# rajan-dubey8/camouflage-multimodal

Measured on AMD Instinct MI355X. Metric: images/sec fwd+bwd (fusion model train step: fwd + loss + bwd + clip + AdamW), higher is better.
Workload: dtype bf16; 1 GPU; BASELINE configs[1] on the path that exists (SURVEY 8d): cross-attention fusion model, packed variable-Nr minibatch (Nr ~ real 303..530 histogram, mean 483), Nk=13 real KG rows, train mode dropout 0.3, random-init weights; batch_per_gpu=16, global_batch=16, rg_dim=128, hidden_dim=256, num_heads=8, parallelism=dp1, precision=bf16 MFMA operands, fp32 accumulate/optimizer

## Files before the change

### camouflage_multimodal_amd/csrc/fused_rows.h

```cpp
#pragma once
#include "common.h"

typedef unsigned short us16;

struct ShadowJob { us16* dst; int N, K, transposed, nsrc; const float* src[4]; int rows[4]; int ld[4]; int chunk_begin; int lo; };
#define SHADOW_MAXJ 24
#define SHADOW_MAXZ 24
struct ShadowBatch { ShadowJob j[SHADOW_MAXJ]; int n; void* zero_ptr[SHADOW_MAXZ]; size_t zero_bytes[SHADOW_MAXZ]; int nzero; };
int launch_weight_shadows(ShadowBatch& sb, hipStream_t stream);

struct FrontStream {
  const float* X; int M;
  const us16* W0; const float* b0;
  const us16* W1; const float* bq; const float* bkv;
  us16* X16;
  us16* R16; us16* Q16; us16* KV16;
  int tile_begin;
};
#define FUSED_FRONT_MAXZ 4
#define FUSED_FRONT_MAXX 20
#define FUSED_BWD1_MAXZ 16
struct FrontArgs {
  FrontStream s[2]; float qscale; int save; unsigned long long* stamps; int exp;
  void* zero_ptr[FUSED_FRONT_MAXZ]; unsigned zero_bytes[FUSED_FRONT_MAXZ]; int nzero;
// ... 55 lines not shown

struct Bwd2Args {
  const us16* Q2_16; const us16* dO2_16; const float* lse2; const float* delta2;
  const us16* KV2_16;
  us16* dQKV16;
  const us16* dU16; const us16* WcRgT; us16* dR16;
  float* dQ2acc;
  const float* dKV;
  const us16* dU2_16; const us16* WcKgT; us16* dQKVkg16; us16* dG16;
  float* dGpart;
  int* tickets;
  const int* off; const int* tile_off; const int4* tile_desc;
  int B, Nk, rg_tiles_max, rows_rg; float qscale; DropCfg drop; unsigned long long* stamps;
  int param_space;
  int split_finish;
};
int launch_fused_bwd2(Bwd2Args& a, int variant, hipStream_t stream);
int launch_wide2_bwd2(Bwd2Args& a, hipStream_t stream);
size_t fused_bwd2_lds();

#define FUSED_PART_FLOATS 544
#define FUSED_MAX_SPLITS 64
size_t fused_front_lds();
size_t fused_back_lds();

#define FUSED_WIDE_MAXSEG 48
int launch_wide_front(FrontArgs& a, int rt, hipStream_t stream, int kg_only = 0);
int launch_wide_rgfwd(const FrontStream& f, float qscale, BackArgs& b, int rt, int max_nr, hipStream_t stream);
int launch_wide_back(BackArgs& a, int rt, int max_nr, hipStream_t stream);
int wide_max_rows(int rt);

// ... 4 lines not shown
```

### camouflage_multimodal_amd/csrc/fused_rows.hip

```cpp
#include "fused_rows.h"
#include "shadow_inl.h"
#include "gemm.h"
#include "mfma_inl.h"

namespace {

template <int NT, int KS, bool W_IS_A, int DEPTH, bool USE_ROT = true>
struct Stage {
  static constexpr int TOTAL = NT * KS;
  static constexpr int D = DEPTH < TOTAL ? DEPTH : TOTAL;
  static_assert(!USE_ROT || (KS & (KS - 1)) == 0, "rotated k order: power-of-two k steps");
  u32x4 buf[D];
  const u32x4* wp; int rot;
  __device__ __forceinline__ int keff(int ks) const { return USE_ROT ? ((ks + rot) & (KS - 1)) : ks; }
  __device__ __forceinline__ const u32x4* wptr(int i) const { return wp + 64 * (keff(i / NT) * NT + (i % NT)); }
  __device__ __forceinline__ void prefetch(const u32x4* __restrict__ wp_, int rot_) {
    wp = wp_; rot = rot_;
#pragma unroll
    for (int i = 0; i < D; ++i) buf[i] = *wptr(i);
  }
  __device__ __forceinline__ void run(const char* act, f32x16 (&acc)[NT]) {
    run_f([&](int ks) { return *reinterpret_cast<const bf16x8*>(act + 32 * ks); }, acc);
  }
  template <class F>
// ... 343 lines not shown
      const float il = invL[hd * 16 + j];
      *reinterpret_cast<u32x2*>(bufO + j * PR + 2 * (32 * hd + 4 * f4)) =
          u32x2{pack2(acc[it][0] * il, acc[it][1] * il), pack2(acc[it][2] * il, acc[it][3] * il)};
    }
  }
}

template <int DEPTH, bool ROT, int OCC>
__global__ __launch_bounds__(256, OCC) void back_kernel(const BackArgs a) {
  extern __shared__ __attribute__((aligned(16))) char smem[];
  const int tid = threadIdx.x, lane = tid & 63, l31 = lane & 31, h = lane >> 5;
  const int w = __builtin_amdgcn_readfirstlane(tid >> 6);
  const int nkg = a.B * a.max_splits;
  const int vid = (int)blockIdx.x < a.lead_tiles ? nkg + (int)blockIdx.x : ((int)blockIdx.x < a.lead_tiles + nkg ? (int)blockIdx.x - a.lead_tiles : (int)blockIdx.x);
  const bool kg = vid < nkg;
  const int rot = ROT ? (int)(blockIdx.x >> 3) : 0;
  using L = BackL<OCC>;
  char* bufO = smem + L::O; char* bufY = smem + L::Y;
  float* red = reinterpret_cast<float*>(smem + L::RED);
  float* tile32 = reinterpret_cast<float*>(smem);
  int b; size_t rowg0; int nrows; float inv_n;
  stamp(a.stamps, 0);
  const BackStream& S = a.s[kg ? 1 : 0];
  Stage<2, 16, true, DEPTH> sto;
  Stage<4, 16, false, DEPTH> stf;
  if (!kg) sto.prefetch(reinterpret_cast<const u32x4*>(S.Wo) + (size_t)w * (16 * 2 * 64) + lane, rot);
  if (kg) {
    b = vid / a.max_splits;
    const int sp = vid - b * a.max_splits;
    const int nsplit = (a.off[b + 1] - a.off[b] + SPLIT_ROWS - 1) / SPLIT_ROWS;
    if (sp >= nsplit) return;
    attn_kg_split(a, smem, b, sp, w, lane);
    stamp(a.stamps, 4);
    asm volatile("s_waitcnt vmcnt(0)" ::: "memory");
    __syncthreads();
    int* flag = reinterpret_cast<int*>(red);
    if (tid == 0) flag[0] = __hip_atomic_fetch_add(a.tickets + b, 1, __ATOMIC_RELAXED, __HIP_MEMORY_SCOPE_AGENT);
    __syncthreads();
    stamp(a.stamps, 5);
    if (flag[0] != nsplit - 1) return;
    if (tid == 0) {
      __builtin_amdgcn_fence(__ATOMIC_ACQUIRE, "agent");
      asm volatile("s_waitcnt vmcnt(0)" ::: "memory");
    }
// ... 491 lines not shown
    se.prefetch(reinterpret_cast<const u32x4*>(a.WcKgT) + (size_t)w * (48 * 2 * 64) + 64 * (16 * 2) + lane, 0);
    for (int c = tid; c < 32 * 64; c += 256) {
      const int j = c >> 6, ch = c & 63;
      u32x4 v = u32x4{0u, 0u, 0u, 0u};
      if (j < Nk) {
        const float* src = a.dKV + (krow0 + j) * 512 + 8 * ch;
        const float4 x0 = *reinterpret_cast<const float4*>(src), x1 = *reinterpret_cast<const float4*>(src + 4);
        v = u32x4{pack2(x0.x, x0.y), pack2(x0.z, x0.w), pack2(x1.x, x1.y), pack2(x1.z, x1.w)};
      }
      *reinterpret_cast<u32x4*>(bufT + j * PQ + 512 + 16 * ch) = v;
    }
    __syncthreads();
    f32x16 acc[2] = {zero16(), zero16()};
    se.run(bufT + l31 * PQ + 512 + 16 * h, acc);
    copy_out<6>(bufT, PQ, 512, a.dQKVkg16 + 256, 768, krow0, Nk);
    if (l31 < Nk) {
#pragma unroll
      for (int t = 0; t < 2; ++t)
#pragma unroll
        for (int g = 0; g < 4; ++g) {
          const int c0 = 64 * w + 32 * t + 8 * g + 4 * h;
          const u32x2 uv = *reinterpret_cast<const u32x2*>(a.dU2_16 + (krow0 + l31) * 256 + c0);
          float* dst = a.dGpart + (krow0 + l31) * 256 + c0;
          __hip_atomic_store(dst, acc[t][4 * g] + bf_lo(uv.x), __ATOMIC_RELAXED, __HIP_MEMORY_SCOPE_AGENT);
          __hip_atomic_store(dst + 1, acc[t][4 * g + 1] + bf_hi(uv.x), __ATOMIC_RELAXED, __HIP_MEMORY_SCOPE_AGENT);
          __hip_atomic_store(dst + 2, acc[t][4 * g + 2] + bf_lo(uv.y), __ATOMIC_RELAXED, __HIP_MEMORY_SCOPE_AGENT);
          __hip_atomic_store(dst + 3, acc[t][4 * g + 3] + bf_hi(uv.y), __ATOMIC_RELAXED, __HIP_MEMORY_SCOPE_AGENT);
        }
    }
  } else {
  const int4 td = a.tile_desc[(int)blockIdx.x - a.B];
// ... 103 lines not shown
    sr.run(bufT + l31 * PQ + 16 * h, acc);
    copy_out<6>(bufT, PQ, 512, a.dQKV16 + 256, 768, rowg0, nrows);
    if (rok) {
#pragma unroll
      for (int t = 0; t < 2; ++t)
#pragma unroll
        for (int g = 0; g < 4; ++g) {
          const int c0 = 64 * w + 32 * t + 8 * g + 4 * h;
          const u32x2 uv = *reinterpret_cast<const u32x2*>(a.dU16 + (rowg0 + l31) * 256 + c0);
          *reinterpret_cast<u32x2*>(a.dR16 + (rowg0 + l31) * 256 + c0) =
              u32x2{pack2(acc[t][4 * g] + bf_lo(uv.x), acc[t][4 * g + 1] + bf_hi(uv.x)), pack2(acc[t][4 * g + 2] + bf_lo(uv.y), acc[t][4 * g + 3] + bf_hi(uv.y))};
        }
    }
  }
  stamp(a.stamps, 2);
  }
  asm volatile("s_waitcnt vmcnt(0)" ::: "memory");
  __syncthreads();
  if (tid == 0) flag[0] = __hip_atomic_fetch_add(a.tickets + b, 1, __ATOMIC_RELAXED, __HIP_MEMORY_SCOPE_AGENT);
  __syncthreads();
  if (flag[0] != a.tile_off[b + 1] - a.tile_off[b]) return;
  Stage<2, 16, true, DEPTH, false> sg;
  sg.prefetch(reinterpret_cast<const u32x4*>(a.WcKgT) + (size_t)w * (48 * 2 * 64) + lane, 0);
  if (tid == 0) {
    __builtin_amdgcn_fence(__ATOMIC_ACQUIRE, "agent");
    asm volatile("s_waitcnt vmcnt(0)" ::: "memory");
  }
  __syncthreads();
  const size_t krow0 = (size_t)b * Nk;
  for (int c = tid; c < 32 * 32; c += 256) {
// ... 305 lines not shown
  const int prof = gemm_prof_open(stream, 2.0 * rows * (512.0 * 256.0 + 256.0 * 256.0) + (kg_only ? 0.0 : 10.0 * (double)a.rows_rg * a.Nk * 256.0), PROF_BWD1);
  if (variant == 0) launch_lds<bwd1_kernel<12, false>>(grid, dim3(256), W_LDS, stream, k);
  else              launch_lds<bwd1_kernel<12, true>>(grid, dim3(256), W_LDS, stream, k);
  gemm_prof_close(prof, stream);
  return (int)hipGetLastError();
}

size_t fused_bwd2_lds() { return X_LDS; }

int launch_fused_bwd2(Bwd2Args& a, int variant, hipStream_t stream) {
  (void)variant;
  if (a.B < 1 || a.Nk < 1 || a.Nk > 16 || a.rg_tiles_max < 1 || !a.Q2_16 || !a.dO2_16 || !a.lse2 || !a.delta2 || !a.KV2_16 || !a.dQKV16 ||
      !a.dU16 || !a.WcRgT || !a.dR16 || !a.dQ2acc || !a.dKV || !a.dU2_16 || !a.WcKgT || !a.dQKVkg16 || !a.dG16 || !a.dGpart || !a.tickets || !a.off || !a.tile_off || !a.tile_desc)
    return (int)hipErrorInvalidValue;
  if (!al16(a.dQKV16) || !al16(a.dQKVkg16) || !al16(a.WcRgT) || !al16(a.WcKgT) || !al16(a.dQ2acc) || !al16(a.dKV)) return (int)hipErrorInvalidValue;
  const double rows = (double)a.rows_rg + (double)a.B * a.Nk;
  const int prof = gemm_prof_open(stream, (a.param_space ? 0.0 : 2.0 * rows * 768.0 * 256.0) + 10.0 * (double)a.rows_rg * a.Nk * 256.0, PROF_BWD2);
  if (!a.param_space) a.split_finish = 0;
  if (!a.param_space) launch_lds<bwd2_kernel<12, false>>(dim3(a.B + a.rg_tiles_max), dim3(256), X_LDS, stream, a);
  else                launch_lds<bwd2p_kernel<12, false>>(dim3(a.B + a.rg_tiles_max), dim3(256), X_LDS, stream, a);
  if (a.split_finish) hipLaunchKernelGGL(bwd2_finish_kernel, dim3(a.B), dim3(256), 0, stream, a);
  gemm_prof_close(prof, stream);
  return (int)hipGetLastError();
}
```

### camouflage_multimodal_amd/csrc/fusion_abi.hip

```cpp
#include <hip/hip_runtime.h>

#include <algorithm>
#include <cmath>
#include <cstdio>
#include <cstring>
#include <string>

#include "../../include/camo_fusion.h"

#include "attn.h"
#include "gemm.h"
#include "fused_rows.h"
#include "tail_wide.h"
#include "attn_maps.h"
#include "gemm16.h"
#include "misc.h"
#include "abi_util.h"

namespace {
thread_local std::string g_err;
}

int camo_abi::fail(int code, const std::string& msg) { g_err = msg; return code; }
int camo_abi::fail_hip(int e, const char* where) {
// ... 805 lines not shown
    t.B = B;
  }
  if (pl.bwd1 == CAMO_BWD1_64) CK(launch_wide2_bwd1(a1, x.opt->fused_variant, st), "fused backward, first half (64-row half-blocks)");
  else                         CK(launch_fused_bwd1(a1, x.opt->fused_variant, st), "fused backward, first half");
  if (pl.tail_event == CAMO_EVENT_AFTER_BWD1) CK(record_tail_event(c, st), "tail event");
  Bwd2Args a2; std::memset(&a2, 0, sizeof(a2));
  a2.Q2_16 = f.Q2_16; a2.dO2_16 = f.dO2_16; a2.lse2 = f.lse2; a2.delta2 = f.delta2; a2.KV2_16 = f.KV2_16; a2.dQKV16 = f.dQKV16;
  a2.dU16 = f.dU16; a2.WcRgT = f.WcRgT; a2.dR16 = f.dR16; a2.dQ2acc = w.dQ2acc; a2.dKV = w.dKV;
  a2.dU2_16 = f.dU2_16; a2.WcKgT = f.WcKgT; a2.dQKVkg16 = f.dQKVkg16; a2.dG16 = f.dG16; a2.dGpart = f.dGpart;
  a2.tickets = w.tickets + B; a2.off = rg_offsets; a2.tile_off = bd.tile_off; a2.tile_desc = bd.tile_desc;
  a2.B = B; a2.Nk = Nk; a2.rows_rg = T; a2.rg_tiles_max = T / 32 + B; a2.qscale = a1.qscale; a2.drop = drop;
  a2.stamps = g_dbg_stamps ? g_dbg_stamps + (size_t)3 * g_dbg_stamp_blocks * 8 : nullptr;
  const bool param_space = pl.param_space != 0;
  a2.param_space = param_space ? 1 : 0;
  a2.split_finish = pl.bwd2 != CAMO_BWD2_ROWS32 ? 1 : 0;
  if (pl.bwd2 == CAMO_BWD2_64) CK(launch_wide2_bwd2(a2, st), "fused backward, second half (64-row blocks)");
  else CK(launch_fused_bwd2(a2, x.opt->fused_variant, st), "fused backward, second half");
  if (!param_space) {
    GB16 g(drop, *x.opt, st);
    g.tn(f.dH16, 2 * H, f.Y16, H, Gr[CAMO_P_F1_W0], H, Gr[CAMO_P_F1_B0], 2 * H, H, T);
    g.tn(f.dU16, H, f.O16, H, Gr[CAMO_P_A1_OUT_W], H, Gr[CAMO_P_A1_OUT_B], H, H, T);
    g.tn(f.dQKV16, 3 * H, f.R16, H, Gr[CAMO_P_A1_IN_W], H, Gr[CAMO_P_A1_IN_B], H, H, T);
    g.tn(f.dQKV16 + H, 3 * H, f.R16, H, Gr[CAMO_P_A2_IN_W] + HH, H, Gr[CAMO_P_A2_IN_B] + H, 2 * H, H, T);
    g.tn(f.dR16, H, f.X16, D, Gr[CAMO_P_RG_PROJ_W], D, Gr[CAMO_P_RG_PROJ_B], H, D, T);
    g.tn(f.dH2_16, 2 * H, f.Y2_16, H, Gr[CAMO_P_F2_W0], H, Gr[CAMO_P_F2_B0], 2 * H, H, TK);
    g.tn(f.dU2_16, H, f.O2_16, H, Gr[CAMO_P_A2_OUT_W], H, Gr[CAMO_P_A2_OUT_B], H, H, TK);
    g.tn(f.dQKVkg16, 3 * H, f.G16, H, Gr[CAMO_P_A2_IN_W], H, Gr[CAMO_P_A2_IN_B], H, H, TK);
    g.tn(f.dQKVkg16 + H, 3 * H, f.G16, H, Gr[CAMO_P_A1_IN_W] + HH, H, Gr[CAMO_P_A1_IN_B] + H, 2 * H, H, TK);
    g.tn(f.dG16, H, f.KG16, D, Gr[CAMO_P_KG_PROJ_W], D, Gr[CAMO_P_KG_PROJ_B], H, D, TK);
    CK(g.run(), "node-level weight gradients");
    return 0;
  }
  float* const Mrg = w.parM; float* const Mkg = Mrg + (size_t)3 * H * D;
  float* const dbrg = Mkg + (size_t)3 * H * D; float* const dbkg = dbrg + 3 * H;
  GB16 g(drop, *x.opt, st);
  g.tn(f.dH16, 2 * H, f.Y16, H, Gr[CAMO_P_F1_W0], H, Gr[CAMO_P_F1_B0], 2 * H, H, T);
  g.tn(f.dU16, H, f.O16, H, Gr[CAMO_P_A1_OUT_W], H, Gr[CAMO_P_A1_OUT_B], H, H, T);
  g.tn(f.dQKV16, 3 * H, f.X16, D, Mrg, D, dbrg, H, D, T).bias_grad2 = Gr[CAMO_P_A1_IN_B];
  g.tn(f.dQKV16 + H, 3 * H, f.X16, D, Mrg + (size_t)H * D, D, dbrg + H, 2 * H, D, T).bias_grad2 = Gr[CAMO_P_A2_IN_B] + H;
  g.tn(f.dU16, H, f.X16, D, Gr[CAMO_P_RG_PROJ_W], D, Gr[CAMO_P_RG_PROJ_B], H, D, T);
  g.tn(f.dH2_16, 2 * H, f.Y2_16, H, Gr[CAMO_P_F2_W0], H, Gr[CAMO_P_F2_B0], 2 * H, H, TK);
  g.tn(f.dU2_16, H, f.O2_16, H, Gr[CAMO_P_A2_OUT_W], H, Gr[CAMO_P_A2_OUT_B], H, H, TK);
  g.tn(f.dQKVkg16, 3 * H, f.KG16, D, Mkg, D, dbkg, H, D, TK).bias_grad2 = Gr[CAMO_P_A2_IN_B];
  g.tn(f.dQKVkg16 + H, 3 * H, f.KG16, D, Mkg + (size_t)H * D, D, dbkg + H, 2 * H, D, TK).bias_grad2 = Gr[CAMO_P_A1_IN_B] + H;
// ... 510 lines not shown
```

### camouflage_multimodal_amd/csrc/gemm.h

```cpp
#pragma once
#include "common.h"

#define GEMM_MAXP 12

enum : int {
  GF_RELU = 1,
  GF_DROPOUT = 2,
  GF_ATOMIC = 4,
  GF_RELU_BWD = 8,
  GF_RES_BCAST = 16,
  GF_SIGMOID = 32,
  GF_A_KMAJOR = 64,
  GF_B_KMAJOR = 128,
  GF_A_VIRT = 256
};

struct GemmProb {
  const float* A; const float* B; float* C;
  const float* bias;
  const float* res;
  float* bias_grad;
  int M, N, K;
  int lda, ldb, ldc, ldr;
  int flags;
  uint32_t drop_site;
  float aux_scale;
  const int* row_sample; const float* inv_nr; int uniform_n;
  int tiles_n, ksplit, kchunk, tile_begin;
};
// ... 18 lines not shown
```

### camouflage_multimodal_amd/csrc/gemm16.h

```cpp
#pragma once
#include "common.h"
#include "gemm.h"

#define GEMM16_MAXP 12

struct Gemm16Prob {
  const unsigned short* A; const unsigned short* B;
  float* C;
  unsigned short* C16;
  const float* bias;
  const float* res;
  float* bias_grad;
  float* bias_grad2;
  int M, N, K;
  int lda, ldb, ldc, ldc16, ldr;
  int flags;
  uint32_t drop_site;
  float aux_scale;
  const int* row_sample; const float* inv_nr; int uniform_n;
  float* colmean; int ldm;
  int ln_mode;
  const float* ln_gamma; const float* ln_beta; float* ln_stats; const float* ln_x; float* ln_dgamma; float* ln_dbeta;
  const float* virt_g; int ldg;
  int tiles_n, ksplit, kchunk, tile_begin;
};

struct Gemm16Batch {
  Gemm16Prob p[GEMM16_MAXP];
  int n;
  DropCfg drop;
  int exp;
  int n_heavy;
};

struct Gemm16Knobs {
  int tn_big = -1;
  int balance = 1;
  int tn_kcap = 0;
// ... 5 lines not shown
```

### camouflage_multimodal_amd/csrc/gemm16.hip

```cpp
#include "gemm16.h"
#include "mfma_inl.h"


namespace {

constexpr int BM = 64, BN = 128, BK = 64;
constexpr int PM = 128;
constexpr int PKA = 192, PKB = 320;
constexpr int A_NT_BYTES = BM * PM;
constexpr int A_TN_BYTES = BK * PKA;
constexpr int NT_BUF_BYTES = (BM + BN) * PM;
constexpr int BUF_BYTES = 32768;

struct Stage { u32x4 a[2], b[4]; };

__device__ __forceinline__ u32x4 virt_chunk(u32x4 act, float4 g0, float4 g1, float scale) {
  auto sel = [&](uint32_t bits, float g) { return __uint_as_float(bits) > 0.f ? g * scale : 0.f; };
  u32x4 o;
  o.x = pack2(sel(act.x << 16, g0.x), sel(act.x & 0xFFFF0000u, g0.y));
  o.y = pack2(sel(act.y << 16, g0.z), sel(act.y & 0xFFFF0000u, g0.w));
  o.z = pack2(sel(act.z << 16, g1.x), sel(act.z & 0xFFFF0000u, g1.y));
  o.w = pack2(sel(act.w << 16, g1.z), sel(act.w & 0xFFFF0000u, g1.w));
  return o;
}

#define G16_PIPELINE_LOOP                                                                      \
  _Pragma("unroll") for (int j = 0; j < PIPE; ++j) gloadi(j, j);                               \
  sstorei(0, 0);                                                                               \
  gloadi(0, PIPE);                                                                             \
// ... 145 lines not shown
        sum = 0.f; cur = sm;
      }
      sum += tile[(half * 32 + r) * TP + t];
    }
    if (one) {
      if (half == 1) hsum[t] = sum;
      __syncthreads();
      if (half == 0 && col < N && cur >= 0)
        atomicAdd(P.colmean + (size_t)cur * P.ldm + col, (sum + hsum[t]) * (P.row_sample ? P.inv_nr[cur] : 1.0f / (float)P.uniform_n));
    } else if (cur >= 0 && col < N) {
      atomicAdd(P.colmean + (size_t)cur * P.ldm + col, sum * (P.row_sample ? P.inv_nr[cur] : 1.0f / (float)P.uniform_n));
    }
  }
}

template <int PIPE, bool VIRT>
__device__ __forceinline__ void body_tn(const Gemm16Prob& P, int m0, int n0, int kt0, int nt, char* smem, int exp = 0) {
  const int tid = threadIdx.x, lane = tid & 63, wave = tid >> 6;
  const int wr = wave >> 1, wc = wave & 1, l31 = lane & 31, h = lane >> 5;
  const int M = P.M, N = P.N;

  uint32_t goa[2], gob[4];
  int la[2], lb[4];
#pragma unroll
  for (int i = 0; i < 2; ++i) {
    const int s = tid + 256 * i, kr = s >> 3, c = s & 7;
    goa[i] = ((uint32_t)kr * (uint32_t)P.lda + (uint32_t)min(m0 + 8 * c, M - 8)) * 2u;
    la[i] = kr * PKA + 16 * c;
  }
#pragma unroll
  for (int i = 0; i < 4; ++i) {
    const int s = tid + 256 * i, kr = s >> 4, c = s & 15;
    gob[i] = ((uint32_t)kr * (uint32_t)P.ldb + (uint32_t)min(n0 + 8 * c, N - 8)) * 2u;
    lb[i] = A_TN_BYTES + kr * PKB + 16 * c;
  }
  const char* Ab = reinterpret_cast<const char*>(P.A);
  const char* Bb = reinterpret_cast<const char*>(P.B);
  const size_t astep = (size_t)BK * P.lda * 2, bstep = (size_t)BK * P.ldb * 2;

  f32x16 acc[2], accb;
#pragma unroll
  for (int r = 0; r < 16; ++r) { acc[0][r] = 0.f; acc[1][r] = 0.f; accb[r] = 0.f; }
  const bool do_bsum = P.bias_grad != nullptr && n0 == 0 && wc == 0;
  const short one = (short)0x3F80;
  const bf16x8 ones = {one, one, one, one, one, one, one, one};
  Stage st[PIPE];
  int sa[PIPE][2];
  float* gs = reinterpret_cast<float*>(smem + 2 * BUF_BYTES);
  if constexpr (VIRT) {
    const int ns = P.uniform_n > 0 && !P.row_sample ? (P.K + P.uniform_n - 1) / P.uniform_n : P.ldc16;
    for (int i = tid; i < ns * 64; i += 256) {
      const int sm = i >> 6, f = i & 63, c = min(m0 + f, M - 1);
      const float inv = P.row_sample ? P.inv_nr[sm] : 1.0f / (float)P.uniform_n;
      gs[i] = P.virt_g[(size_t)sm * P.ldg + c] * inv * P.aux_scale;
    }
    __syncthreads();
  }

  auto gload = [&](Stage& r, int (&srow)[2], int kt) {
    const int k = kt0 + min(kt, nt - 1);
    const char* a = Ab + (size_t)k * astep;
    const char* b = Bb + (size_t)k * bstep;
#pragma unroll
    for (int i = 0; i < 2; ++i) r.a[i] = *reinterpret_cast<const u32x4*>(a + goa[i]);
#pragma unroll
    for (int i = 0; i < 4; ++i) r.b[i] = *reinterpret_cast<const u32x4*>(b + gob[i]);
    if constexpr (VIRT) {
#pragma unroll
      for (int i = 0; i < 2; ++i) {
        const int node = min(k * BK + ((tid + 256 * i) >> 3), P.K - 1);
        srow[i] = P.row_sample ? P.row_sample[node] : node / P.uniform_n;
      }
    }
  };
  auto sstore = [&](const Stage& r, const int (&srow)[2], int buf) {
    char* base = smem + buf * BUF_BYTES;
#pragma unroll
    for (int i = 0; i < 2; ++i) {
      u32x4 a = r.a[i];
      if constexpr (VIRT) {
        const float* g = gs + srow[i] * 64 + 8 * ((tid + 256 * i) & 7);
        a = virt_chunk(a, *reinterpret_cast<const float4*>(g), *reinterpret_cast<const float4*>(g + 4), 1.0f);
      }
      *reinterpret_cast<u32x4*>(base + la[i]) = a;
    }
#pragma unroll
    for (int i = 0; i < 4; ++i) *reinterpret_cast<u32x4*>(base + lb[i]) = r.b[i];
  };
  const int g = (lane >> 4) & 1, q = (lane >> 2) & 3, p = lane & 3;
  const int fa = (8 * h + q) * PKA + 64 * wr + 32 * g + 8 * p;
  const int fb = A_TN_BYTES + (8 * h + q) * PKB + 128 * wc + 32 * g + 8 * p;
  auto compute = [&](int buf) {
    const char* base = smem + buf * BUF_BYTES;
#pragma unroll
// ... 3 lines not shown
      const s16x4 a0 = lds_tr16(pa), a1 = lds_tr16(pa + 4 * PKA);
      const s16x4 b00 = lds_tr16(pb), b01 = lds_tr16(pb + 4 * PKB);
      const s16x4 b10 = lds_tr16(pb + 64), b11 = lds_tr16(pb + 64 + 4 * PKB);
      const bf16x8 a = {a0.x, a0.y, a0.z, a0.w, a1.x, a1.y, a1.z, a1.w};
      const bf16x8 b0 = {b00.x, b00.y, b00.z, b00.w, b01.x, b01.y, b01.z, b01.w};
      const bf16x8 b1 = {b10.x, b10.y, b10.z, b10.w, b11.x, b11.y, b11.z, b11.w};
      acc[0] = __builtin_amdgcn_mfma_f32_32x32x16_bf16(a, b0, acc[0], 0, 0, 0);
      acc[1] = __builtin_amdgcn_mfma_f32_32x32x16_bf16(a, b1, acc[1], 0, 0, 0);
      if (do_bsum) accb = __builtin_amdgcn_mfma_f32_32x32x16_bf16(a, ones, accb, 0, 0, 0);
    }
  };
  auto gloadi = [&](int j, int kt) { gload(st[j], sa[j], kt); };
  auto sstorei = [&](int j, int buf) { sstore(st[j], sa[j], buf); };
  G16_PIPELINE_LOOP

  const int rowb = m0 + wr * 32 + 4 * h;
  if ((exp & 1) && acc[0][0] != 12345.f) return;
  if (do_bsum && l31 == 0) {
#pragma unroll
    for (int r = 0; r < 16; ++r) {
      const int row = rowb + (r & 3) + 8 * (r >> 2);
      if (row < M) { atomicAdd(P.bias_grad + row, accb[r]); if (P.bias_grad2) atomicAdd(P.bias_grad2 + row, accb[r]); }
    }
  }
#pragma unroll
  for (int j = 0; j < 2; ++j) {
    const int col = n0 + wc * 64 + j * 32 + l31;
    if (col >= N) continue;
    float* cp = P.C + col;
#pragma unroll
// ... 221 lines not shown
  }
  int pi = 0;
#pragma unroll
  for (int i = 1; i < GEMM16_MAXP; ++i)
    if (i < gb.n && bid >= gb.p[i].tile_begin) pi = i;
  const Gemm16Prob& P = gb.p[pi];
  int t = bid - P.tile_begin;
  if constexpr (ROWS) {
    if (P.ln_mode) {
      if (P.flags & GF_A_VIRT) body_nt_row<PIPE, true>(gb, P, t * RM, smem_raw);
      else                     body_nt_row<PIPE, false>(gb, P, t * RM, smem_raw);
      return;
    }
  }
  const int tiles = ((P.M + BM - 1) / BM) * P.tiles_n;
  const int ks = t / tiles; t -= ks * tiles;
  const int tn = t % P.tiles_n, tm = t / P.tiles_n;
  if (P.flags & GF_A_KMAJOR) {
    const int ktiles = (P.K + 127) / 128 * 2;
    const int per = P.kchunk / BK, kt0 = ks * per;
    if constexpr (ROWS) {
      if (P.flags & GF_A_VIRT) { body_tn<PIPE, true>(P, tm * BM, tn * BN, kt0, min(per, ktiles - kt0), smem_raw); return; }
    }
    body_tn<PIPE, false>(P, tm * BM, tn * BN, kt0, (gb.exp & 2) ? 2 : min(per, ktiles - kt0), smem_raw, gb.exp);
  } else {
    body_nt<PIPE>(gb, P, tm * BM, tn * BN, smem_raw);
  }
}

constexpr int GM = 128, GN = 256;
constexpr int GPA = 320, GPB = 576;
constexpr int GA_BYTES = BK * GPA;
constexpr int GBUF_BYTES = GA_BYTES + BK * GPB;

template <int PIPE>
// ... 100 lines not shown
    }
#pragma unroll
    for (int j = 0; j < 2; ++j) {
      const int col = n0 + 64 * wc + 32 * j + l31;
      if (col >= N) continue;
      float* cp = P.C + col;
#pragma unroll
      for (int r = 0; r < 16; ++r) {
        const int row = rowb + (r & 3) + 8 * (r >> 2);
        if (row < M) atomicAdd(cp + (size_t)row * P.ldc, acc[i][j][r]);
      }
    }
  }
}

constexpr int KCAP_MIN = 8;
bool al16(const void* p) { return (reinterpret_cast<uintptr_t>(p) & 15) == 0; }

}

static int launch_tnbig(Gemm16Batch& gb, const Gemm16Knobs& kn, hipStream_t stream) {
  int total = 0;
  static const int kcaps[] = {512, 384, 256, 192, 128, 96, 64, 48, 32, 24, 16, 12, 8, 6, 4};
  for (int ci = 0;; ++ci) {
    const int kcap = kn.tn_kcap > 0 ? kn.tn_kcap : kcaps[ci];
    total = 0;
    for (int i = 0; i < gb.n; ++i) {
      Gemm16Prob& p = gb.p[i];
      if (p.M < 8 || p.N < 8 || p.K < 1 || !p.C || p.C16 || p.bias || p.res || !al16(p.A) || !al16(p.B) || (p.lda & 7) || (p.ldb & 7))
        return (int)hipErrorInvalidValue;
// ... 12 lines not shown
  gb.n_heavy = 0; gb.exp = kn.exp;
  double fl = 0.0;
  for (int i = 0; i < gb.n; ++i) fl += 2.0 * gb.p[i].M * (double)gb.p[i].N * gb.p[i].K;
  const int prof = gemm_prof_open(stream, fl);
  launch_lds<gemm16_tnbig_kernel<2>>(dim3(total), dim3(512), 2 * GBUF_BYTES, stream, gb, total);
  gemm_prof_close(prof, stream);
  return (int)hipGetLastError();
}
int launch_gemm16_batch(Gemm16Batch& gb, const Gemm16Knobs& kn, hipStream_t stream) {
  if (gb.n <= 0) return 0;
  if (gb.n > GEMM16_MAXP) return (int)hipErrorInvalidValue;
  {
    bool all_tn = true; int kmax = 0;
    for (int i = 0; i < gb.n; ++i) {
      const Gemm16Prob& p = gb.p[i];
      all_tn = all_tn && (p.flags & GF_A_KMAJOR) && (p.flags & GF_B_KMAJOR) && !(p.flags & GF_A_VIRT) && !p.ln_mode && (p.M % 8) == 0 && (p.N % 8) == 0;
      kmax = p.K > kmax ? p.K : kmax;
    }
    const bool big = kn.tn_big < 0 ? kmax >= 40000 : kn.tn_big > 0;
    if (all_tn && big) return launch_tnbig(gb, kn, stream);
  }
  int total = 0, kcap_used = 0;
  static const int kcaps[] = {512, 384, 256, 192, 128, 96, 64, 48, 32, 24, 16, 8};
  for (int ci = 0;; ++ci) {
    const int kcap = kn.tn_kcap > 0 ? kn.tn_kcap : kcaps[ci];
    total = 0; kcap_used = kcap;
    for (int i = 0; i < gb.n; ++i) {
      Gemm16Prob& p = gb.p[i];
      const bool akm = p.flags & GF_A_KMAJOR, bkm = p.flags & GF_B_KMAJOR;
      if (akm != bkm || p.M < 1 || p.N < 1 || p.K < 1) return (int)hipErrorInvalidValue;
      if (!al16(p.A) || !al16(p.B) || (p.lda & 7) || (p.ldb & 7)) return (int)hipErrorInvalidValue;
      if ((double)(akm ? p.K + 128 : p.M) * p.lda * 2.0 >= 4.0e9 || (double)(akm ? p.K + 128 : p.N) * p.ldb * 2.0 >= 4.0e9)
        return (int)hipErrorInvalidValue;
      p.tiles_n = (p.N + BN - 1) / BN;
      int tiles = ((p.M + BM - 1) / BM) * p.tiles_n;
      if (p.ln_mode) {
        if (akm || p.N != RN || !p.ln_gamma || !al16(p.ln_gamma) || (p.ln_mode == 1 && (!p.ln_beta || !al16(p.ln_beta))) ||
            (p.ln_mode == 2 && (!p.ln_x || !al16(p.ln_x) || !p.ln_stats || !p.ln_dgamma || !p.ln_dbeta)) ||
            (p.flags & (GF_RELU | GF_DROPOUT | GF_RELU_BWD)))
          return (int)hipErrorInvalidValue;
        p.tiles_n = 1;
        tiles = (p.M + RM - 1) / RM;
      }
      if (akm) {
        if ((p.M & 7) || (p.N & 7) || p.M < 8 || p.N < 8 || !p.C || p.C16 || p.bias || p.res ||
            (p.flags & ~(GF_A_KMAJOR | GF_B_KMAJOR | GF_ATOMIC | GF_A_VIRT)))
          return (int)hipErrorInvalidValue;
        if (p.flags & GF_A_VIRT) {
          const int ns = p.row_sample ? p.ldc16 : (p.uniform_n > 0 ? (p.K + p.uniform_n - 1) / p.uniform_n : 0);
          if (!p.virt_g || ns < 1 || ns * 256 > 2 * ROW_BUF_BYTES - 2 * BUF_BYTES || (!p.row_sample && p.uniform_n < 1))
            return (int)hipErrorInvalidValue;
        }
        const int ktiles = (p.K + 127) / 128 * 2;
        const int per = ktiles < kcap ? ktiles : kcap;
        p.kchunk = per * BK;
        p.ksplit = (ktiles + per - 1) / per;
      } else {
        if ((p.K % BK) || (p.N & 3) || (p.flags & (GF_ATOMIC | GF_SIGMOID)) || p.bias_grad) return (int)hipErrorInvalidValue;
        if ((p.C && (!al16(p.C) || (p.ldc & 3))) || (p.C16 && ((reinterpret_cast<uintptr_t>(p.C16) & 7) || (p.ldc16 & 3))) ||
            (p.bias && !al16(p.bias)) || (p.res && (!al16(p.res) || (p.ldr & 3))) || (p.colmean && !p.row_sample && p.uniform_n < 1))
          return (int)hipErrorInvalidValue;
        p.kchunk = p.K; p.ksplit = 1;
      }
      p.tile_begin = total;
      total += tiles * p.ksplit;
    }
    if (kn.tn_kcap > 0 || (kcap > 16 ? total >= 440 : total >= 200) || kcap <= KCAP_MIN) break;
  }
  gb.n_heavy = 0; gb.exp = kn.exp;
  if (kn.balance && kcap_used <= 16) {
    int i = 0;
    while (i < gb.n && (gb.p[i].flags & GF_A_KMAJOR) && gb.p[i].ksplit > 1) ++i;
    const int first_light = i;
    while (i < gb.n && (gb.p[i].flags & GF_A_KMAJOR) && gb.p[i].ksplit == 1) ++i;
    if (i == gb.n && first_light > 0 && first_light < gb.n) gb.n_heavy = gb.p[first_light].tile_begin;
  }
  bool has_tn = false, has_rows = false, has_virt = false;
  for (int i = 0; i < gb.n; ++i) {
    has_tn = has_tn || (gb.p[i].flags & GF_A_KMAJOR); has_rows = has_rows || gb.p[i].ln_mode;
    has_virt = has_virt || (gb.p[i].flags & GF_A_VIRT);
    if ((gb.p[i].flags & GF_A_VIRT) && !(gb.p[i].flags & GF_A_KMAJOR) && (!gb.p[i].ln_mode || !gb.p[i].virt_g || (gb.p[i].ldg & 3)))
      return (int)hipErrorInvalidValue;
  }
  if (has_virt && !has_rows) return (int)hipErrorInvalidValue;
  double fl = 0.0;
  for (int i = 0; i < gb.n; ++i) fl += 2.0 * gb.p[i].M * (double)gb.p[i].N * gb.p[i].K;
  const int prof = gemm_prof_open(stream, fl);
  if (!has_rows && !has_tn) hipLaunchKernelGGL((gemm16_kernel<2, false>), dim3(total), dim3(256), 2 * NT_BUF_BYTES, stream, gb, total);
  else if (!has_rows)       launch_lds<gemm16_kernel<2, false>>(dim3(total), dim3(256), 2 * BUF_BYTES, stream, gb, total);
  else                      launch_lds<gemm16_kernel<2, true>>(dim3(total), dim3(256), 2 * ROW_BUF_BYTES, stream, gb, total);
  gemm_prof_close(prof, stream);
  return (int)hipGetLastError();
}
```

Before: 94360 images/s.

## Defer KG query-gradient projection from bwd2 into the weight-gradient GEMM batch

In the second backward kernel, the per-sample KG blocks now write a partial dG (dU2 plus the K/V part) and return early when deferral is enabled, instead of running the query-projection step serially. The deferred work moves into the batched weight-gradient GEMM. A new fp32-A path converts dQ2acc on the fly and computes the query input-projection weight gradient, with an epilogue that folds in the KG projection-weight gradient via atomics. Extra row tiles finish dG and write the bf16 dQ. This shortens the critical path of bwd2 at the cost of more complex GEMM tiles, extra atomics and a second pass over dG; the kg-split rotation now uses the sample index.

```diff
diff --git a/camouflage_multimodal_amd/csrc/fused_rows.h b/camouflage_multimodal_amd/csrc/fused_rows.h
--- a/camouflage_multimodal_amd/csrc/fused_rows.h
+++ b/camouflage_multimodal_amd/csrc/fused_rows.h
@@ -93,7 +93,9 @@
   int B, Nk, rg_tiles_max, rows_rg; float qscale; DropCfg drop; unsigned long long* stamps;
   int param_space;
   int split_finish;
+  int kg_defer;
 };
+#define FUSED_BWD2_DEFER_MAX_TK 512
 int launch_fused_bwd2(Bwd2Args& a, int variant, hipStream_t stream);
 int launch_wide2_bwd2(Bwd2Args& a, hipStream_t stream);
 size_t fused_bwd2_lds();
diff --git a/camouflage_multimodal_amd/csrc/fused_rows.hip b/camouflage_multimodal_amd/csrc/fused_rows.hip
--- a/camouflage_multimodal_amd/csrc/fused_rows.hip
+++ b/camouflage_multimodal_amd/csrc/fused_rows.hip
@@ -381,7 +381,7 @@
   const int nkg = a.B * a.max_splits;
   const int vid = (int)blockIdx.x < a.lead_tiles ? nkg + (int)blockIdx.x : ((int)blockIdx.x < a.lead_tiles + nkg ? (int)blockIdx.x - a.lead_tiles : (int)blockIdx.x);
   const bool kg = vid < nkg;
-  const int rot = ROT ? (int)(blockIdx.x >> 3) : 0;
+  int rot = ROT ? (int)(blockIdx.x >> 3) : 0;
   using L = BackL<OCC>;
   char* bufO = smem + L::O; char* bufY = smem + L::Y;
   float* red = reinterpret_cast<float*>(smem + L::RED);
@@ -395,6 +395,7 @@
   if (kg) {
     b = vid / a.max_splits;
     const int sp = vid - b * a.max_splits;
+    if (ROT) rot = b;
     const int nsplit = (a.off[b + 1] - a.off[b] + SPLIT_ROWS - 1) / SPLIT_ROWS;
     if (sp >= nsplit) return;
     attn_kg_split(a, smem, b, sp, w, lane);
@@ -916,7 +917,24 @@
     f32x16 acc[2] = {zero16(), zero16()};
     se.run(bufT + l31 * PQ + 512 + 16 * h, acc);
     copy_out<6>(bufT, PQ, 512, a.dQKVkg16 + 256, 768, krow0, Nk);
-    if (l31 < Nk) {
+    if (a.kg_defer) {
+      us16* const dGp16 = reinterpret_cast<us16*>(a.dGpart);
+      if (l31 < Nk) {
+#pragma unroll
+        for (int t = 0; t < 2; ++t)
+#pragma unroll
+          for (int g = 0; g < 4; ++g) {
+            const int c0 = 64 * w + 32 * t + 8 * g + 4 * h;
+            const u32x2 uv = *reinterpret_cast<const u32x2*>(a.dU2_16 + (krow0 + l31) * 256 + c0);
+            *reinterpret_cast<u32x2*>(dGp16 + (krow0 + l31) * 256 + c0) =
+                u32x2{pack2(acc[t][4 * g] + bf_lo(uv.x), acc[t][4 * g + 1] + bf_hi(uv.x)), pack2(acc[t][4 * g + 2] + bf_lo(uv.y), acc[t][4 * g + 3] + bf_hi(uv.y))};
+          }
+      }
+      if (b == a.B - 1) {
+        const size_t tk = (size_t)a.B * Nk, n16 = (((tk + 127) & ~size_t(127)) - tk) * 32;
+        for (size_t c = tid; c < n16; c += 256) *(reinterpret_cast<u32x4*>(dGp16 + tk * 256) + c) = u32x4{0u, 0u, 0u, 0u};
+      }
+    } else if (l31 < Nk) {
 #pragma unroll
       for (int t = 0; t < 2; ++t)
 #pragma unroll
@@ -1050,6 +1068,11 @@
     }
   }
   stamp(a.stamps, 2);
+  }
+  if (a.kg_defer) {
+    if (early) { stamp(a.stamps, 1); stamp(a.stamps, 2); }
+    stamp(a.stamps, 3);
+    return;
   }
   asm volatile("s_waitcnt vmcnt(0)" ::: "memory");
   __syncthreads();
@@ -1385,8 +1408,10 @@
       !a.dU16 || !a.WcRgT || !a.dR16 || !a.dQ2acc || !a.dKV || !a.dU2_16 || !a.WcKgT || !a.dQKVkg16 || !a.dG16 || !a.dGpart || !a.tickets || !a.off || !a.tile_off || !a.tile_desc)
     return (int)hipErrorInvalidValue;
   if (!al16(a.dQKV16) || !al16(a.dQKVkg16) || !al16(a.WcRgT) || !al16(a.WcKgT) || !al16(a.dQ2acc) || !al16(a.dKV)) return (int)hipErrorInvalidValue;
-  const double rows = (double)a.rows_rg + (double)a.B * a.Nk;
-  const int prof = gemm_prof_open(stream, (a.param_space ? 0.0 : 2.0 * rows * 768.0 * 256.0) + 10.0 * (double)a.rows_rg * a.Nk * 256.0, PROF_BWD2);
+  if (a.param_space) a.kg_defer = 0;
+  else if (a.kg_defer < 0) a.kg_defer = a.B * a.Nk <= FUSED_BWD2_DEFER_MAX_TK ? 1 : 0;
+  const double dr = 2.0 * ((double)a.rows_rg * 768.0 + (double)a.B * a.Nk * (a.kg_defer ? 512.0 : 768.0)) * 256.0;
+  const int prof = gemm_prof_open(stream, (a.param_space ? 0.0 : dr) + 10.0 * (double)a.rows_rg * a.Nk * 256.0, PROF_BWD2);
   if (!a.param_space) a.split_finish = 0;
   if (!a.param_space) launch_lds<bwd2_kernel<12, false>>(dim3(a.B + a.rg_tiles_max), dim3(256), X_LDS, stream, a);
   else                launch_lds<bwd2p_kernel<12, false>>(dim3(a.B + a.rg_tiles_max), dim3(256), X_LDS, stream, a);
diff --git a/camouflage_multimodal_amd/csrc/fusion_abi.hip b/camouflage_multimodal_amd/csrc/fusion_abi.hip
--- a/camouflage_multimodal_amd/csrc/fusion_abi.hip
+++ b/camouflage_multimodal_amd/csrc/fusion_abi.hip
@@ -843,10 +843,18 @@
   const bool param_space = pl.param_space != 0;
   a2.param_space = param_space ? 1 : 0;
   a2.split_finish = pl.bwd2 != CAMO_BWD2_ROWS32 ? 1 : 0;
+  a2.kg_defer = x.opt->exp == 32 ? 0 : (x.opt->exp == 64 ? 1 : (x.opt->tn_big > 0 ? 0 : -1));
   if (pl.bwd2 == CAMO_BWD2_64) CK(launch_wide2_bwd2(a2, st), "fused backward, second half (64-row blocks)");
   else CK(launch_fused_bwd2(a2, x.opt->fused_variant, st), "fused backward, second half");
   if (!param_space) {
     GB16 g(drop, *x.opt, st);
+    const bool kgq = a2.kg_defer == 1;
+    if (kgq) {
+      Gemm16Prob& p = g.tn(nullptr, H, f.KG16, D, Gr[CAMO_P_KG_PROJ_W], D, Gr[CAMO_P_KG_PROJ_B], H, D, TK);
+      p.A = reinterpret_cast<const us*>(w.dQ2acc); p.flags |= GF_A_F32 | GF_KGQ;
+      p.kgq_wT = f.WcKgT; p.kgq_w = P[CAMO_P_A2_IN_W]; p.ldg = H;
+      p.C16 = f.dG16; p.ldc16 = H; p.kgq_part16 = reinterpret_cast<const us*>(f.dGpart); p.kgq_a16 = f.dQKVkg16; p.kgq_lda16 = 3 * H;
+    }
     g.tn(f.dH16, 2 * H, f.Y16, H, Gr[CAMO_P_F1_W0], H, Gr[CAMO_P_F1_B0], 2 * H, H, T);
     g.tn(f.dU16, H, f.O16, H, Gr[CAMO_P_A1_OUT_W], H, Gr[CAMO_P_A1_OUT_B], H, H, T);
     g.tn(f.dQKV16, 3 * H, f.R16, H, Gr[CAMO_P_A1_IN_W], H, Gr[CAMO_P_A1_IN_B], H, H, T);
@@ -854,9 +862,14 @@
     g.tn(f.dR16, H, f.X16, D, Gr[CAMO_P_RG_PROJ_W], D, Gr[CAMO_P_RG_PROJ_B], H, D, T);
     g.tn(f.dH2_16, 2 * H, f.Y2_16, H, Gr[CAMO_P_F2_W0], H, Gr[CAMO_P_F2_B0], 2 * H, H, TK);
     g.tn(f.dU2_16, H, f.O2_16, H, Gr[CAMO_P_A2_OUT_W], H, Gr[CAMO_P_A2_OUT_B], H, H, TK);
-    g.tn(f.dQKVkg16, 3 * H, f.G16, H, Gr[CAMO_P_A2_IN_W], H, Gr[CAMO_P_A2_IN_B], H, H, TK);
+    if (kgq) {
+      Gemm16Prob& p = g.tn(nullptr, H, f.G16, H, Gr[CAMO_P_A2_IN_W], H, Gr[CAMO_P_A2_IN_B], H, H, TK);
+      p.A = reinterpret_cast<const us*>(w.dQ2acc); p.flags |= GF_A_F32;
+    } else {
+      g.tn(f.dQKVkg16, 3 * H, f.G16, H, Gr[CAMO_P_A2_IN_W], H, Gr[CAMO_P_A2_IN_B], H, H, TK);
+    }
     g.tn(f.dQKVkg16 + H, 3 * H, f.G16, H, Gr[CAMO_P_A1_IN_W] + HH, H, Gr[CAMO_P_A1_IN_B] + H, 2 * H, H, TK);
-    g.tn(f.dG16, H, f.KG16, D, Gr[CAMO_P_KG_PROJ_W], D, Gr[CAMO_P_KG_PROJ_B], H, D, TK);
+    g.tn(kgq ? reinterpret_cast<const us*>(f.dGpart) : f.dG16, H, f.KG16, D, Gr[CAMO_P_KG_PROJ_W], D, Gr[CAMO_P_KG_PROJ_B], H, D, TK);
     CK(g.run(), "node-level weight gradients");
     return 0;
   }
diff --git a/camouflage_multimodal_amd/csrc/gemm.h b/camouflage_multimodal_amd/csrc/gemm.h
--- a/camouflage_multimodal_amd/csrc/gemm.h
+++ b/camouflage_multimodal_amd/csrc/gemm.h
@@ -12,7 +12,9 @@
   GF_SIGMOID = 32,
   GF_A_KMAJOR = 64,
   GF_B_KMAJOR = 128,
-  GF_A_VIRT = 256
+  GF_A_VIRT = 256,
+  GF_A_F32 = 512,
+  GF_KGQ = 1024
 };
 
 struct GemmProb {
diff --git a/camouflage_multimodal_amd/csrc/gemm16.h b/camouflage_multimodal_amd/csrc/gemm16.h
--- a/camouflage_multimodal_amd/csrc/gemm16.h
+++ b/camouflage_multimodal_amd/csrc/gemm16.h
@@ -22,6 +22,8 @@
   int ln_mode;
   const float* ln_gamma; const float* ln_beta; float* ln_stats; const float* ln_x; float* ln_dgamma; float* ln_dbeta;
   const float* virt_g; int ldg;
+  const unsigned short* kgq_wT; const float* kgq_w;
+  const unsigned short* kgq_part16; unsigned short* kgq_a16; int kgq_lda16;
   int tiles_n, ksplit, kchunk, tile_begin;
 };
 
diff --git a/camouflage_multimodal_amd/csrc/gemm16.hip b/camouflage_multimodal_amd/csrc/gemm16.hip
--- a/camouflage_multimodal_amd/csrc/gemm16.hip
+++ b/camouflage_multimodal_amd/csrc/gemm16.hip
@@ -1,5 +1,6 @@
 #include "gemm16.h"
 #include "mfma_inl.h"
+#include <type_traits>
 
 
 namespace {
@@ -13,6 +14,7 @@
 constexpr int BUF_BYTES = 32768;
 
 struct Stage { u32x4 a[2], b[4]; };
+struct StageF { float4 a[4]; u32x4 b[4]; int ok; };
 
 __device__ __forceinline__ u32x4 virt_chunk(u32x4 act, float4 g0, float4 g1, float scale) {
   auto sel = [&](uint32_t bits, float g) { return __uint_as_float(bits) > 0.f ? g * scale : 0.f; };
@@ -188,8 +190,90 @@
   }
 }
 
-template <int PIPE, bool VIRT>
-__device__ __forceinline__ void body_tn(const Gemm16Prob& P, int m0, int n0, int kt0, int nt, char* smem, int exp = 0) {
+__device__ __forceinline__ void kgq_finish(const Gemm16Prob& P, int m0, int q, const f32x16 (&acc)[2], const f32x16& accb, char* smem) {
+  const int tid = threadIdx.x, lane = tid & 63, wave = tid >> 6;
+  const int wr = wave >> 1, wc = wave & 1, l31 = lane & 31, h = lane >> 5;
+  constexpr int PT = 144;
+  const u32x4* wp = reinterpret_cast<const u32x4*>(P.kgq_wT) + ((size_t)(q * 48 + (m0 >> 4)) * 2 + wr) * 64 + lane;
+  u32x4 wf[4];
+#pragma unroll
+  for (int s = 0; s < 4; ++s) wf[s] = wp[128 * s];
+  float* sv = reinterpret_cast<float*>(smem + 128 * PT);
+#pragma unroll
+  for (int j = 0; j < 2; ++j) {
+    char* row = smem + (64 * wc + 32 * j + l31) * PT + 2 * (32 * wr + 4 * h);
+#pragma unroll
+    for (int g = 0; g < 4; ++g)
+      *reinterpret_cast<u32x2*>(row + 16 * g) = u32x2{pack2(acc[j][4 * g], acc[j][4 * g + 1]), pack2(acc[j][4 * g + 2], acc[j][4 * g + 3])};
+  }
+  if (wc == 0 && l31 == 0) {
+#pragma unroll
+    for (int r = 0; r < 16; ++r) sv[32 * wr + acc_row(r, h)] = accb[r];
+  }
+  __syncthreads();
+  f32x16 o[2] = {zero16(), zero16()};
+#pragma unroll
+  for (int s = 0; s < 4; ++s) {
+    const char* pb = smem + (64 * wc + l31) * PT + 32 * s + 16 * h;
+    const bf16x8 b0 = *reinterpret_cast<const bf16x8*>(pb), b1 = *reinterpret_cast<const bf16x8*>(pb + 32 * PT);
+    o[0] = __builtin_amdgcn_mfma_f32_32x32x16_bf16(as_frag(wf[s]), b0, o[0], 0, 0, 0);
+    o[1] = __builtin_amdgcn_mfma_f32_32x32x16_bf16(as_frag(wf[s]), b1, o[1], 0, 0, 0);
+  }
+#pragma unroll
+  for (int j = 0; j < 2; ++j) {
+    float* cp = P.C + 64 * wc + 32 * j + l31;
+#pragma unroll
+    for (int r = 0; r < 16; ++r) atomicAdd(cp + (size_t)(64 * q + 32 * wr + acc_row(r, h)) * P.ldc, o[j][r]);
+  }
+  {
+    const int i = tid & 63, j0 = 16 * (tid >> 6);
+    const float* w = P.kgq_w + (size_t)(m0 + j0) * P.ldg + 64 * q + i;
+    float sum = 0.f;
+#pragma unroll
+    for (int j = 0; j < 16; ++j) sum = fmaf(w[(size_t)j * P.ldg], sv[j0 + j], sum);
+    atomicAdd(P.bias_grad + 64 * q + i, sum);
+  }
+}
+
+__device__ __forceinline__ void kgq_rows(const Gemm16Prob& P, int r0, char* smem) {
+  const int tid = threadIdx.x, lane = tid & 63, w = tid >> 6, l31 = lane & 31, h = lane >> 5;
+  constexpr int PR_ = 528;
+  for (int c = tid; c < 32 * 32; c += 256) {
+    const int j = c >> 5, ch = c & 31, row = r0 + j;
+    u32x4 v = u32x4{0u, 0u, 0u, 0u};
+    if (row < P.K) {
+      const float* src = reinterpret_cast<const float*>(P.A) + (size_t)row * P.lda + 8 * ch;
+      const float4 x0 = *reinterpret_cast<const float4*>(src), x1 = *reinterpret_cast<const float4*>(src + 4);
+      v = u32x4{pack2(x0.x, x0.y), pack2(x0.z, x0.w), pack2(x1.x, x1.y), pack2(x1.z, x1.w)};
+      *reinterpret_cast<u32x4*>(P.kgq_a16 + (size_t)row * P.kgq_lda16 + 8 * ch) = v;
+    }
+    *reinterpret_cast<u32x4*>(smem + j * PR_ + 16 * ch) = v;
+  }
+  __syncthreads();
+  const u32x4* wp = reinterpret_cast<const u32x4*>(P.kgq_wT) + (size_t)w * (48 * 2 * 64) + lane;
+  f32x16 acc[2] = {zero16(), zero16()};
+#pragma unroll 4
+  for (int ks = 0; ks < 16; ++ks) {
+    const bf16x8 x = *reinterpret_cast<const bf16x8*>(smem + l31 * PR_ + 32 * ks + 16 * h);
+    acc[0] = __builtin_amdgcn_mfma_f32_32x32x16_bf16(as_frag(wp[64 * (2 * ks)]), x, acc[0], 0, 0, 0);
+    acc[1] = __builtin_amdgcn_mfma_f32_32x32x16_bf16(as_frag(wp[64 * (2 * ks + 1)]), x, acc[1], 0, 0, 0);
+  }
+  const int row = r0 + l31;
+  if (row < P.K) {
+#pragma unroll
+    for (int t = 0; t < 2; ++t)
+#pragma unroll
+      for (int g = 0; g < 4; ++g) {
+        const int c0 = 64 * w + 32 * t + 8 * g + 4 * h;
+        const u32x2 pv = *reinterpret_cast<const u32x2*>(P.kgq_part16 + (size_t)row * P.ldc16 + c0);
+        *reinterpret_cast<u32x2*>(P.C16 + (size_t)row * P.ldc16 + c0) =
+            u32x2{pack2(acc[t][4 * g] + bf_lo(pv.x), acc[t][4 * g + 1] + bf_hi(pv.x)), pack2(acc[t][4 * g + 2] + bf_lo(pv.y), acc[t][4 * g + 3] + bf_hi(pv.y))};
+      }
+  }
+}
+
+template <int PIPE, bool VIRT, bool F32A = false>
+__device__ __forceinline__ void body_tn(const Gemm16Prob& P, int m0, int n0, int kt0, int nt, char* smem, int exp = 0, int rq = 0) {
   const int tid = threadIdx.x, lane = tid & 63, wave = tid >> 6;
   const int wr = wave >> 1, wc = wave & 1, l31 = lane & 31, h = lane >> 5;
   const int M = P.M, N = P.N;
@@ -218,7 +302,7 @@
   const bool do_bsum = P.bias_grad != nullptr && n0 == 0 && wc == 0;
   const short one = (short)0x3F80;
   const bf16x8 ones = {one, one, one, one, one, one, one, one};
-  Stage st[PIPE];
+  std::conditional_t<F32A, StageF, Stage> st[PIPE];
   int sa[PIPE][2];
   float* gs = reinterpret_cast<float*>(smem + 2 * BUF_BYTES);
   if constexpr (VIRT) {
@@ -231,12 +315,23 @@
     __syncthreads();
   }
 
-  auto gload = [&](Stage& r, int (&srow)[2], int kt) {
+  auto gload = [&](auto& r, int (&srow)[2], int kt) {
     const int k = kt0 + min(kt, nt - 1);
     const char* a = Ab + (size_t)k * astep;
     const char* b = Bb + (size_t)k * bstep;
-#pragma unroll
-    for (int i = 0; i < 2; ++i) r.a[i] = *reinterpret_cast<const u32x4*>(a + goa[i]);
+    if constexpr (F32A) {
+      r.ok = 0;
+#pragma unroll
+      for (int i = 0; i < 2; ++i) {
+        const int s = tid + 256 * i, row = k * BK + (s >> 3);
+        const float* src = reinterpret_cast<const float*>(P.A) + (size_t)min(row, P.K - 1) * P.lda + min(m0 + 8 * (s & 7), M - 8);
+        r.a[2 * i] = *reinterpret_cast<const float4*>(src); r.a[2 * i + 1] = *reinterpret_cast<const float4*>(src + 4);
+        r.ok |= row < P.K ? 1 << i : 0;
+      }
+    } else {
+#pragma unroll
+      for (int i = 0; i < 2; ++i) r.a[i] = *reinterpret_cast<const u32x4*>(a + goa[i]);
+    }
 #pragma unroll
     for (int i = 0; i < 4; ++i) r.b[i] = *reinterpret_cast<const u32x4*>(b + gob[i]);
     if constexpr (VIRT) {
@@ -247,11 +342,18 @@
       }
     }
   };
-  auto sstore = [&](const Stage& r, const int (&srow)[2], int buf) {
+  auto sstore = [&](const auto& r, const int (&srow)[2], int buf) {
     char* base = smem + buf * BUF_BYTES;
 #pragma unroll
     for (int i = 0; i < 2; ++i) {
-      u32x4 a = r.a[i];
+      u32x4 a;
+      if constexpr (F32A) {
+        const float4 x0 = r.a[2 * i], x1 = r.a[2 * i + 1];
+        a = u32x4{pack2(x0.x, x0.y), pack2(x0.z, x0.w), pack2(x1.x, x1.y), pack2(x1.z, x1.w)};
+        if (!(r.ok >> i & 1)) a = u32x4{0u, 0u, 0u, 0u};
+      } else {
+        a = r.a[i];
+      }
       if constexpr (VIRT) {
         const float* g = gs + srow[i] * 64 + 8 * ((tid + 256 * i) & 7);
         a = virt_chunk(a, *reinterpret_cast<const float4*>(g), *reinterpret_cast<const float4*>(g + 4), 1.0f);
@@ -285,6 +387,9 @@
   auto sstorei = [&](int j, int buf) { sstore(st[j], sa[j], buf); };
   G16_PIPELINE_LOOP
 
+  if constexpr (F32A) {
+    if (P.flags & GF_KGQ) { kgq_finish(P, m0, rq, acc, accb, smem); return; }
+  }
   const int rowb = m0 + wr * 32 + 4 * h;
   if ((exp & 1) && acc[0][0] != 12345.f) return;
   if (do_bsum && l31 == 0) {
@@ -536,11 +641,17 @@
     }
   }
   const int tiles = ((P.M + BM - 1) / BM) * P.tiles_n;
+  if ((P.flags & GF_KGQ) && t >= tiles * P.ksplit) { kgq_rows(P, (t - tiles * P.ksplit) * 32, smem_raw); return; }
   const int ks = t / tiles; t -= ks * tiles;
   const int tn = t % P.tiles_n, tm = t / P.tiles_n;
   if (P.flags & GF_A_KMAJOR) {
     const int ktiles = (P.K + 127) / 128 * 2;
     const int per = P.kchunk / BK, kt0 = ks * per;
+    if (P.flags & GF_A_F32) {
+      if (P.flags & GF_KGQ) body_tn<PIPE, false, true>(P, tm * BM, 0, 0, ktiles, smem_raw, 0, ks);
+      else                  body_tn<PIPE, false, true>(P, tm * BM, tn * BN, kt0, min(per, ktiles - kt0), smem_raw);
+      return;
+    }
     if constexpr (ROWS) {
       if (P.flags & GF_A_VIRT) { body_tn<PIPE, true>(P, tm * BM, tn * BN, kt0, min(per, ktiles - kt0), smem_raw); return; }
     }
@@ -671,6 +782,7 @@
   }
 }
 
+static_assert(sizeof(Gemm16Batch) + sizeof(int) <= 4096, "gemm16_kernel's arguments: the kernel-argument segment is 4 KB");
 constexpr int KCAP_MIN = 8;
 bool al16(const void* p) { return (reinterpret_cast<uintptr_t>(p) & 15) == 0; }
 
@@ -713,7 +825,7 @@
     bool all_tn = true; int kmax = 0;
     for (int i = 0; i < gb.n; ++i) {
       const Gemm16Prob& p = gb.p[i];
-      all_tn = all_tn && (p.flags & GF_A_KMAJOR) && (p.flags & GF_B_KMAJOR) && !(p.flags & GF_A_VIRT) && !p.ln_mode && (p.M % 8) == 0 && (p.N % 8) == 0;
+      all_tn = all_tn && (p.flags & GF_A_KMAJOR) && (p.flags & GF_B_KMAJOR) && !(p.flags & (GF_A_VIRT | GF_A_F32)) && !p.ln_mode && (p.M % 8) == 0 && (p.N % 8) == 0;
       kmax = p.K > kmax ? p.K : kmax;
     }
     const bool big = kn.tn_big < 0 ? kmax >= 40000 : kn.tn_big > 0;
@@ -724,6 +836,7 @@
   for (int ci = 0;; ++ci) {
     const int kcap = kn.tn_kcap > 0 ? kn.tn_kcap : kcaps[ci];
     total = 0; kcap_used = kcap;
+    int extra = 0;
     for (int i = 0; i < gb.n; ++i) {
       Gemm16Prob& p = gb.p[i];
       const bool akm = p.flags & GF_A_KMAJOR, bkm = p.flags & GF_B_KMAJOR;
@@ -742,8 +855,13 @@
         tiles = (p.M + RM - 1) / RM;
       }
       if (akm) {
-        if ((p.M & 7) || (p.N & 7) || p.M < 8 || p.N < 8 || !p.C || p.C16 || p.bias || p.res ||
-            (p.flags & ~(GF_A_KMAJOR | GF_B_KMAJOR | GF_ATOMIC | GF_A_VIRT)))
+        if ((p.M & 7) || (p.N & 7) || p.M < 8 || p.N < 8 || !p.C || (p.C16 && !(p.flags & GF_KGQ)) || p.bias || p.res ||
+            (p.flags & ~(GF_A_KMAJOR | GF_B_KMAJOR | GF_ATOMIC | GF_A_VIRT | GF_A_F32 | GF_KGQ)))
+          return (int)hipErrorInvalidValue;
+        if ((p.flags & GF_A_F32) && ((p.flags & GF_A_VIRT) || (double)p.K * p.lda * 4.0 >= 4.0e9)) return (int)hipErrorInvalidValue;
+        if ((p.flags & GF_KGQ) && (!(p.flags & GF_A_F32) || p.M != 256 || p.N != BN || !p.kgq_wT || !al16(p.kgq_wT) || !p.kgq_w || p.ldg < 256 || !p.bias_grad ||
+                                   !p.C16 || !p.kgq_part16 || !p.kgq_a16 || (reinterpret_cast<uintptr_t>(p.C16) & 7) || (reinterpret_cast<uintptr_t>(p.kgq_part16) & 7) ||
+                                   !al16(p.kgq_a16) || p.ldc16 < 256 || (p.ldc16 & 3) || p.kgq_lda16 < 256 || (p.kgq_lda16 & 7)))
           return (int)hipErrorInvalidValue;
         if (p.flags & GF_A_VIRT) {
           const int ns = p.row_sample ? p.ldc16 : (p.uniform_n > 0 ? (p.K + p.uniform_n - 1) / p.uniform_n : 0);
@@ -754,6 +872,7 @@
         const int per = ktiles < kcap ? ktiles : kcap;
         p.kchunk = per * BK;
         p.ksplit = (ktiles + per - 1) / per;
+        if (p.flags & GF_KGQ) { p.kchunk = ktiles * BK; p.ksplit = 4; extra += tiles * 4 + (p.K + 31) / 32; }
       } else {
         if ((p.K % BK) || (p.N & 3) || (p.flags & (GF_ATOMIC | GF_SIGMOID)) || p.bias_grad) return (int)hipErrorInvalidValue;
         if ((p.C && (!al16(p.C) || (p.ldc & 3))) || (p.C16 && ((reinterpret_cast<uintptr_t>(p.C16) & 7) || (p.ldc16 & 3))) ||
@@ -762,9 +881,9 @@
         p.kchunk = p.K; p.ksplit = 1;
       }
       p.tile_begin = total;
-      total += tiles * p.ksplit;
-    }
-    if (kn.tn_kcap > 0 || (kcap > 16 ? total >= 440 : total >= 200) || kcap <= KCAP_MIN) break;
+      total += tiles * p.ksplit + ((p.flags & GF_KGQ) ? (p.K + 31) / 32 : 0);
+    }
+    if (kn.tn_kcap > 0 || (kcap > 16 ? total - extra >= 440 : total - extra >= 200) || kcap <= KCAP_MIN) break;
   }
   gb.n_heavy = 0; gb.exp = kn.exp;
   if (kn.balance && kcap_used <= 16) {
@@ -783,7 +902,11 @@
   }
   if (has_virt && !has_rows) return (int)hipErrorInvalidValue;
   double fl = 0.0;
-  for (int i = 0; i < gb.n; ++i) fl += 2.0 * gb.p[i].M * (double)gb.p[i].N * gb.p[i].K;
+  for (int i = 0; i < gb.n; ++i) {
+    const Gemm16Prob& p = gb.p[i];
+    if (p.flags & GF_KGQ) fl += 2.0 * p.M * (double)p.N * (4.0 * p.K + 256.0) + 2.0 * p.K * 256.0 * 256.0;
+    else fl += 2.0 * p.M * (double)p.N * p.K;
+  }
   const int prof = gemm_prof_open(stream, fl);
   if (!has_rows && !has_tn) hipLaunchKernelGGL((gemm16_kernel<2, false>), dim3(total), dim3(256), 2 * NT_BUF_BYTES, stream, gb, total);
   else if (!has_rows)       launch_lds<gemm16_kernel<2, false>>(dim3(total), dim3(256), 2 * BUF_BYTES, stream, gb, total);
```

Result: faster. 97440 images/s, median of 6 (+3.3%).
